# fmidev/RoadSurf

Measured on AMD Instinct MI355X. Metric: point_timesteps_per_s, higher is better.
Workload: dtype f64

## Files before the change

roadsurf_amd/csrc/rs_api.hip:

```cpp
#include <hip/hip_runtime.h>
#include <atomic>
#include <cmath>
#include <cstdarg>
#include <cstdio>
#include <cstdlib>
#include <cstring>
#include <mutex>
#include <utility>
#include <vector>

#include "../../include/roadsurf.h"
#include "rs_kernels.h"
#include "rs_ens_table.hpp"
#include "rs_period_rule.hpp"
#include "rs_devutil.hpp"
#include <cstdint>
#include <algorithm>
#include "rs_consts_dev.h"
#include "rs_state.h"

static thread_local char g_err[512] = "";

static int set_err(const char *fmt, ...) {
  va_list ap;
// ... 1282 lines not shown
  dst->wave_tab_valid = false;
  return 0;
}

int rs_hip_clock_probe(int32_t device, void *out, uint32_t spin_us, void *stream) {
  if (!out) return set_err("rs_hip_clock_probe: null output");
  HIP_OK(hipSetDevice(device));
  HIP_OK(rs_launch_clock_probe(static_cast<uint64_t *>(out), spin_us, (hipStream_t)stream));
  return 0;
}

int64_t rs_hip_failed_count(RsPlan *pl) {
  if (!pl) return -1;
  if (hipSetDevice(pl->device) != hipSuccess) return -1;
  unsigned long long h = 0;
  if (pl->f32) {
    std::vector<float> row((size_t)pl->np_pad);
    if (hipMemcpyAsync(row.data(), (const char *)pl->state + (size_t)RS_ST_FAILED * pl->np_pad * sizeof(float),
                       row.size() * sizeof(float), hipMemcpyDeviceToHost, pl->stream) != hipSuccess)
      return -1;
    if (hipStreamSynchronize(pl->stream) != hipSuccess) return -1;
    for (int64_t q = 0; q < pl->npoints; ++q) h += row[(size_t)q] != 0.f ? 1 : 0;
    return (int64_t)h;
  }
  if (hipMemsetAsync(pl->counter, 0, sizeof(h), pl->stream) != hipSuccess) return -1;
  if (rs_launch_count_failed(pl->state, pl->np_pad, pl->npoints, pl->counter, pl->stream) !=
      hipSuccess)
    return -1;
  if (hipMemcpyAsync(&h, pl->counter, sizeof(h), hipMemcpyDeviceToHost, pl->stream) != hipSuccess)
    return -1;
  if (hipStreamSynchronize(pl->stream) != hipSuccess) return -1;
  return (int64_t)h;
}

int rs_hip_first_failed_index(RsPlan *pl, int32_t *out) {
  if (!pl || !out) return set_err("rs_hip_first_failed_index: bad arguments");
  HIP_OK(hipSetDevice(pl->device));
  const size_t esz = pl->f32 ? sizeof(float) : sizeof(double);
  std::vector<char> row((size_t)pl->np_pad * esz);
  HIP_OK(hipMemcpyAsync(row.data(), (const char *)pl->state + (size_t)RS_ST_FAILED * pl->np_pad * esz,
                        row.size(), hipMemcpyDeviceToHost, pl->stream));
  std::vector<int32_t> order;
  if (pl->order) {
    order.resize((size_t)pl->np_pad);
    HIP_OK(hipMemcpyAsync(order.data(), pl->order, order.size() * sizeof(int32_t), hipMemcpyDeviceToHost,
                          pl->stream));
  }
  HIP_OK(hipStreamSynchronize(pl->stream));
  for (int64_t s = 0; s < pl->npoints; ++s) {
    const double v = pl->f32 ? (double)reinterpret_cast<const float *>(row.data())[s]
                             : reinterpret_cast<const double *>(row.data())[s];
    const int64_t p = pl->order ? order[(size_t)s] : s;
    if (p >= 0 && p < pl->npoints) out[p] = (int32_t)v;
  }
  return 0;
}

int rs_hip_sync(RsPlan *pl) {
  if (!pl) return set_err("rs_hip_sync: null plan");
  HIP_OK(hipSetDevice(pl->device));
  HIP_OK(hipStreamSynchronize(pl->stream));
  return 0;
}

static int64_t div_mismatch(RsPlan *pl, int which) {
  if (!pl) return -1;
  if (hipSetDevice(pl->device) != hipSuccess) return -1;
  unsigned long long n[3] = {0, 0, 0};
  if (rs_read_div_mismatch(n, pl->stream) != hipSuccess) return -1;
  return which == 1 ? (int64_t)(n[1] + n[2]) : (int64_t)n[0];
}
int64_t rs_hip_div_mismatch_count(RsPlan *pl) { return div_mismatch(pl, 0); }
int64_t rs_hip_div_special_count(RsPlan *pl) { return div_mismatch(pl, 1); }
int rs_hip_div_samples(RsPlan *pl, double *out) {
  if (!pl || !out) return set_err("rs_hip_div_samples: bad arguments");
  HIP_OK(hipSetDevice(pl->device));
  HIP_OK(rs_read_div_samples(out, pl->stream));
  return 0;
}

int rs_hip_bl_stats(RsPlan *pl, int64_t *out) {
  if (!pl || !out) return set_err("rs_hip_bl_stats: bad arguments");
  HIP_OK(hipSetDevice(pl->device));
  unsigned long long v[57];
  HIP_OK(rs_read_bl_stats(v, pl->stream));
  for (int k = 0; k < 57; ++k) out[k] = (int64_t)v[k];
  return 0;
}

int rs_hip_division_mode(void) {
#if defined(RS_IEEE_DIV)
  return 0;
#elif defined(RS_DIV_CHECK)
  return 2;
#else
  return 1;
#endif
}

int rs_hip_test_math(RsPlan *pl, int32_t fn, int64_t n, const double *x, double *y) {
  if (!pl || !x || !y || n < 1 || fn < 0 || fn > 3) return set_err("rs_hip_test_math: bad arguments");
  HIP_OK(hipSetDevice(pl->device));
  HIP_OK(rs_launch_math_test(fn, n, x, y, pl->stream));
  return 0;
}

int rs_hip_synth_knots(RsPlan *pl, const RsSynthSpec *spec, double *knots, int32_t k0,
                       int32_t nknots) {
  if (!pl || !spec || !knots || nknots < 1 || k0 < 0)
    return set_err("rs_hip_synth_knots: bad arguments");
  if (nknots > 65535) return set_err("rs_hip_synth_knots: at most 65535 knots per call");
  HIP_OK(hipSetDevice(pl->device));
  rs::KnotArgs a;
  a.spec = *spec;
  a.knots = knots;
  a.npoints = pl->npoints;
  a.np_pad = pl->np_pad;
  a.k0 = k0;
  HIP_OK(rs_launch_knots(a, nknots, pl->stream));
  return 0;
}

static int expand_forcing(RsPlan *pl, const RsSynthSpec *spec, const double *knots, int32_t k0,
                          int32_t nknots, const RsForcing *f, int32_t t0, int32_t nsteps, void *stream,
                          const int32_t *gather) {
  if (!pl || !spec || !knots || !f) return set_err("rs_hip_expand_forcing: bad arguments");
  if (check_forcing(pl, f, "rs_hip_expand_forcing")) return -1;
  if (nsteps < 1 || nsteps > 65535 || t0 < 1)
    return set_err("rs_hip_expand_forcing: 1 <= nsteps <= 65535, t0 >= 1");
  const int32_t spk = spec->steps_per_knot;
  if (spk < 1) return set_err("rs_hip_expand_forcing: steps_per_knot < 1");
  const int32_t kfirst = (t0 - 1) / spk;
  const int32_t tlast = t0 + nsteps - 2;
  const int32_t klast = tlast / spk + ((tlast % spk) ? 1 : 0);
  if (kfirst < k0 || klast >= k0 + nknots)
    return set_err("rs_hip_expand_forcing: need knots %d..%d, buffer has %d..%d", kfirst, klast,
                   k0, k0 + nknots - 1);
  if (f->hour_pstride) return set_err("rs_hip_expand_forcing: hour must be a shared axis");
  HIP_OK(hipSetDevice(pl->device));
  rs::ExpandArgs a;
  a.f = *f;
  a.knots = knots;
  a.npoints = pl->npoints;
  a.np_pad = pl->np_pad;
  a.k0 = k0;
  a.t0 = t0;
  a.spk = spk;
  a.start_hour = spec->start_hour;
  a.kfirst = kfirst;
  a.nsteps = nsteps;
  a.r_spk = 1.0 / (double)spk;
  a.gather = gather;
  if (pl->f32) {
    if (f->depth) return set_err("rs_hip_expand_forcing: fp32 windows carry no depth stream");
    HIP_OK(rs32_launch_expand(a, (t0 + nsteps - 2) / spk - kfirst + 1, (hipStream_t)stream));
  } else {
    HIP_OK(rs_launch_expand(a, (t0 + nsteps - 2) / spk - kfirst + 1, (hipStream_t)stream));
  }
  return 0;
}

int rs_hip_expand_forcing_on(RsPlan *pl, const RsSynthSpec *spec, const double *knots, int32_t k0,
                             int32_t nknots, const RsForcing *f, int32_t t0, int32_t nsteps,
                             void *stream) {
  return expand_forcing(pl, spec, knots, k0, nknots, f, t0, nsteps, stream, nullptr);
}

int rs_hip_expand_forcing(RsPlan *pl, const RsSynthSpec *spec, const double *knots, int32_t k0,
                          int32_t nknots, const RsForcing *f, int32_t t0, int32_t nsteps) {
// ... 14 lines not shown
```

roadsurf_amd/csrc/rs_consts_dev.h:

```cpp
#pragma once
#include <cmath>
#include <cstdlib>
#include "../../include/roadsurf.h"

struct RsConstantsDev : RsConstants {
  double meltDen;
  double r_3600, r_3364, r_1000, r_IceMax, r_twoDT, r_DTSecs, r_meltDen, r_logUstar, r_logCond;
  int32_t bareFastOk;
  int32_t precFastOk;
  double chk[8];
  const double *relax_tab;
  const double *cpl_tab;
  double capDZF[RS_MAX_LAYERS + 2];
  double hs1F;
  double hcw[8];
  struct LayerRow {
    double capDZF, condDZ, DyC, dryCap, WCont, pad[3];
  } lk[RS_MAX_LAYERS + 2];
  double stabSafe;
};

static inline double rs_stab_safe(double logMom, double logHeat) {
  if (!(logMom > 0.0 && logMom < HUGE_VAL && logHeat > 0.0 && logHeat < HUGE_VAL)) return NAN;
  const double psih = std::fmin(logHeat / 2.0, logMom / 1.2);
  const double sq = 2.0 * std::exp(psih / 2.0) - 1.0;
  return (1.0 - sq * sq) / 16.0;
}

static inline void rs_consts_dev_fill(const RsConstants &c, RsConstantsDev &d) {
  static_cast<RsConstants &>(d) = c;
  d.meltDen = c.WatMHeat * c.WatDens;
  d.r_3600 = 1.0 / 3600.0;
  d.r_3364 = 1.0 / 3364.0;
  d.r_1000 = 1.0 / 1000.0;
  d.r_IceMax = 1.0 / 1.5;
  d.r_twoDT = 1.0 / c.twoDT;
  d.r_DTSecs = 1.0 / c.DTSecs;
  d.r_meltDen = 1.0 / d.meltDen;
  d.r_logUstar = 1.0 / c.logUstar;
  d.r_logCond = 1.0 / c.logCond;
  const float chk[8] = {100.0f, -0.1f, -90.0f, 120.0f, -1.0f, 4000.0f, 1000.0f, 500.0f};
  for (int i = 0; i < 8; ++i) d.chk[i] = (double)chk[i];
  d.relax_tab = nullptr;
  d.cpl_tab = nullptr;
  for (int j = 0; j < RS_MAX_LAYERS + 2; ++j) {
    d.lk[j].capDZF = 0.0;
    d.lk[j].condDZ = c.condDZ[j];
    d.lk[j].DyC = c.DyC[j];
    d.lk[j].dryCap = c.dryCap[j];
    d.lk[j].WCont = c.WCont[j];
    d.lk[j].pad[0] = d.lk[j].pad[1] = d.lk[j].pad[2] = 0.0;
  }
  {
    const float h[8] = {-0.0050f, 0.0079f, 1000.0028f, 0.0000102f, 0.0017169f, 0.11516f, 3.4739f, 4217.2f};
    for (int i = 0; i < 8; ++i) d.hcw[i] = (double)h[i];
  }
  for (int j = 0; j < RS_MAX_LAYERS + 2; ++j) d.capDZF[j] = 0.0;
  d.hs1F = 0.0;
  for (int j = 1; j <= c.NLayers && j <= RS_MAX_LAYERS; ++j) {
    const volatile double chwt = 920.0 * 2100.0;
    const volatile double wc = c.WCont[j] * chwt;
    const volatile double vsh = c.dryCap[j] + wc;
    const volatile double den = c.DyC[j] * vsh;
    d.capDZF[j] = -(1.0 / den);
    d.lk[j].capDZF = d.capDZF[j];
    if (j == 1) {
      const volatile double num = vsh * c.HSfac1;
      d.hs1F = num / c.twoDT;
    }
  }
  d.stabSafe = rs_stab_safe(c.logMom, c.logHeat);
  d.bareFastOk = (c.MaxWatmms >= 0.0 && c.MaxSnowmms >= 0.0 && c.MaxIcemms >= 0.0 && c.MaxDepmms >= 0.0) ? 1 : 0;
  d.precFastOk = (c.MinPrecmm >= 0.0) ? 1 : 0;
}

static inline const char *rs_consts_domain_error(const RsConstants &c) {
  const double lo = 1e-30, hi = 1e30;
  auto pos = [&](double x) { return x > lo && x < hi; };
  auto mag = [&](double x) { return (x > lo && x < hi) || (x < -lo && x > -hi); };
  if (!pos(c.DTSecs) || !pos(c.twoDT)) return "DTSecs";
  if (!mag(c.logUstar)) return "logUstar = log(ZRefW/ZMom)";
  if (!mag(c.logCond)) return "logCond = log(ZRefT/ZHeat)";
  if (!(c.logMom > -hi && c.logMom < hi) || !(c.logHeat > -hi && c.logHeat < hi)) return "logMom/logHeat";
  if (!pos(c.VK_Const)) return "VK_Const";
  if (!pos(c.LVap) || !pos(c.LFus)) return "LVap/LFus";
  if (!pos(c.WatMHeat * c.WatDens)) return "WatMHeat*WatDens";
  if (!pos(c.HSfac1)) return "layer grid (ZDpth(2)-ZDpth(1))";
  for (int j = 1; j <= c.NLayers; ++j) {
    if (!pos(c.DyC[j])) return "DyC (layer grid)";
    if (!(c.dryCap[j] >= 0.0) || !(c.WCont[j] >= 0.0) || !pos(c.dryCap[j] + c.WCont[j] * 1.9e6))
      return "layer heat capacity (vsh/Poro/WCont)";
    if (!(c.ZDpth[j + 1] - c.ZDpth[j] > lo)) return "layer grid (ZDpth)";
  }
  return nullptr;
}

#include <cmath>
#include <vector>
static inline std::vector<double> rs_decay_table(const RsConstants &c, bool on, double den) {
  std::vector<double> t;
  const double dt = c.DTSecs;
  if (!on || !(dt == std::floor(dt)) || !(dt * ((double)c.SimLen + 1.0) < 9.0e15)) return t;
  t.resize((size_t)c.SimLen + 1);
  for (int32_t d = 0; d <= c.SimLen; ++d) t[(size_t)d] = std::exp(-((dt * d) - (dt * 0)) / den);
  return t;
}
static inline std::vector<double> rs_relax_table(const RsConstants &c) {
  return rs_decay_table(c, c.use_relaxation != 0, (double)(4.f * 3600.f));
}
static inline std::vector<double> rs_cpl_table(const RsConstants &c) {
  return rs_decay_table(c, c.use_coupling != 0 && c.cplReduction > 1e-30 && c.cplReduction < 1e30,
                        c.cplReduction);
}
```

roadsurf_amd/csrc/rs_kernels.hip:

```cpp
#include <hip/hip_runtime.h>
#include <cstdlib>
#include "rs_physics.hpp"
#include "rs_state.h"
#include "rs_synth.h"
#include "rs_kernels.h"

#ifndef RS_CPL_WAVES
#define RS_CPL_WAVES 2
#endif
#ifndef RS_REGIME_WINDOW
#define RS_REGIME_WINDOW 30
#endif

namespace rs {

constexpr int kBlock = RS_BLOCK;

typedef RsConstantsDev __attribute__((address_space(4))) ConstsAS;
template <class Args>
__device__ __forceinline__ const ConstsAS &consts_of(Args a) {
  return *(const ConstsAS *)a->consts;
}

template <int NL, int NREG>
// ... 729 lines not shown
        } else {
          s.tsurf = (T.get(1) + T.get(2)) / R4(2.0);
        }
      }
      const double tair = q.tair;
      auto qs = q;
      if (SKY) {
        const int64_t row = (int64_t)k * ka->f.t_stride + row0;
        const LaneOff L(lane);
        double sw_dir = L.ld(ka->f.sw_dir + row), lw_net = L.ld(ka->f.lw_net + row);
        if (i < c.SimLen) {
          if (sky_on && sky_limits_bad(sw_dir, lw_net)) fail_at(i);
          sw_dir = sky_clamp_direct(sw_dir, q.sw);
        }
        if (sky_on) {
          int64_t hstride;
          const double *hrow = horizon_row(ka, sky.hcol, hstride);
          if (!sky_view_radiation(ka->f.sun + (int64_t)k * RS_SUN_COLS, sky.sinlat, sky.coslat, sky.lonrad, sky.coslon,
                                  sky.sinlon, sky.skyv, ka->pp.albedo_surroundings, hrow, hstride, qs.sw, sw_dir, qs.lw,
                                  lw_net))
            fail_at(i);
        }
        sky_write_back(ka, k, row0, sky_on, sw_dir, qs.sw, qs.lw, [&](double *base, double v) { L.st(base, v); });
      }
      const Fluxes fx = model_step_fluxes_prepped<SCORE ? 1 : 2>(c, mt, s, qs, cp);
      if (SCORE) {
        score += (fx.trips & 63) - 5;
        if ((fx.trips & 64) && k >= nsteps - RS_REGIME_WINDOW) score |= 1 << 30;
      } else if (k == nsteps - 1) {
        score = fx.trips;
      }
      if (LATE) t3 = mail.v[k & 1][1][ml];
      model_step_ground<RegProfile<2>, RegProfile<2>, false>(c, s, T, t3, tair, fx, R4(-9999.9), cp);
      if (owrite) {
        if (OUTIDX && ka->out_index) store_outputs<true, false>(ka, orow, row0, lane, s, true);
        else store_outputs<false, true>(ka, orow, row0, lane, s, true);
      }
      if (s.failed) blank_rows(REPLAY && cpl_ce + 1 > i + 1 ? cpl_ce + 1 : i + 1);
      if (CPL && cpl_on && i < c.SimLen && i == cpl_ce)
        cpl_window_end(ka->state, ka->np_pad, row0 + lane, cw, s, cpl_swcorr, cpl_lwcorr, cpl_lastobs, parked);
    }
    mail.failed[(k & 1) ^ 1][ml] = (s.failed || (CPL && (parked || (i + 1) != next_i))) ? 1u : 0u;
    mail.v[(k & 1) ^ 1][0][ml] = T.get(2);
    if (!OUTIDX) {
      if (owrite) {
        orow_next += ostride;
        owait = odec - 1;
      } else {
        --owait;
      }
    }
    duo_meet();
  }
  if (CPL && live) a.state[(int64_t)RS_ST_CPL_RESUME * a.np_pad + p] = (double)next_i;
  if (live) {
    double *st = a.state;
    const int64_t np = a.np_pad;
    uint32_t le = ml;
    if (LATE) asm volatile("" : "+v"(le));
    const int64_t p = LATE ? row0 + le : row0 + lane;
    st[(int64_t)(RS_ST_TMP0 + 0) * np + p] = T.get(1);
    st[(int64_t)(RS_ST_TMP0 + 1) * np + p] = T.get(2);
    st[(int64_t)RS_ST_TNW1 * np + p] = s.tnw1;
    st[(int64_t)RS_ST_TNW2 * np + p] = s.tnw2;
    st[(int64_t)RS_ST_TSURF * np + p] = s.tsurf;
    st[(int64_t)RS_ST_WAT * np + p] = s.wat;
    st[(int64_t)RS_ST_SNOW * np + p] = s.snow;
    st[(int64_t)RS_ST_ICE * np + p] = s.ice;
    st[(int64_t)RS_ST_ICE2 * np + p] = s.ice2;
    st[(int64_t)RS_ST_DEP * np + p] = s.dep;
    st[(int64_t)RS_ST_Q2MELT * np + p] = s.q2melt;
    st[(int64_t)RS_ST_T4MELT * np + p] = s.t4melt;
    st[(int64_t)RS_ST_ALBEDO * np + p] = s.albedo;
    st[(int64_t)RS_ST_VERYCOLD * np + p] = s.verycold ? 1.0 : 0.0;
    st[(int64_t)RS_ST_BLSCORE * np + p] = SCORE ? bl_score_key(score, s) : (double)score;
  }
}

template <bool FULL>
struct KnotLerp {
  double v0[FULL ? 7 : 6], dv[FULL ? 7 : 6];
  int32_t ph1;
  int32_t spk, k, r, hour, night;
  double span, r_spk;
};
template <bool FULL>
__device__ __forceinline__ void knot_begin(KernArgs ka, KnotLerp<FULL> &K, int32_t i0) {
  K.spk = ka->spk;
  {
    const uint64_t u = (uint64_t)__double_as_longlong((double)K.spk);
    const uint32_t lo = __builtin_amdgcn_readfirstlane((uint32_t)u), hi = __builtin_amdgcn_readfirstlane((uint32_t)(u >> 32));
    K.span = __longlong_as_double((long long)(((uint64_t)hi << 32) | lo));
  }
  K.r_spk = ka->r_spk;
  const int32_t t = i0 - 1;
  K.k = __builtin_amdgcn_readfirstlane(t / K.spk);
  K.r = t - K.k * K.spk;
  K.hour = 0;
  K.night = 0;
}
template <bool FULL>
__device__ __forceinline__ Forcing knot_forcing(KernArgs ka, int64_t col, bool live, KnotLerp<FULL> &K,
                                                int32_t &kcur, int32_t i) {
  const int32_t k = K.k, r = K.r;
  int32_t ph0 = 0;
  if (k != kcur) {
    kcur = k;
    const ConstsAS &c = consts_of(ka);
    K.hour = (k + ka->start_hour) % 24;
    const bool night = ((double)K.hour >= c.NightOn) || ((double)K.hour <= c.NightOff);
    K.night = __builtin_amdgcn_readfirstlane(night ? 1 : 0);
    const int fld[7] = {0, 2, 3, 4, 5, 6, 1};
    const int64_t np = ka->np_pad;
    const double *ka_ = ka->knots + ((int64_t)(k - ka->knot_k0) * RS_KNOT_FIELDS) * np + col;
    const bool has_b = (k + 1 - ka->knot_k0) < ka->knot_n;
    const double *kb_ = ka_ + (int64_t)RS_KNOT_FIELDS * np;
#pragma unroll
    for (int q = 0; q < (FULL ? 7 : 6); ++q) {
      K.v0[q] = live ? ka_[(int64_t)fld[q] * np] : 0.0;
      const double v1 = (live && has_b) ? kb_[(int64_t)fld[q] * np] : K.v0[q];
      K.dv[q] = v1 - K.v0[q];
    }
    ph0 = live ? (int32_t)ka_[8 * np] : 0;
    K.ph1 = (live && has_b) ? (int32_t)kb_[8 * np] : ph0;
  }
  const int32_t spk = FULL ? ka->spk : K.spk;
  const double secs = (double)r, span = FULL ? (double)spk : K.span, r_spk = FULL ? ka->r_spk : K.r_spk;
  Forcing f;
  f.tair = K.v0[0] + rs_div_u(secs * K.dv[0], span, r_spk);
  f.vz = K.v0[1] + rs_div_u(secs * K.dv[1], span, r_spk);
  f.rhz = K.v0[2] + rs_div_u(secs * K.dv[2], span, r_spk);
  f.prec = K.v0[3] + rs_div_u(secs * K.dv[3], span, r_spk);
  f.sw = K.v0[4] + rs_div_u(secs * K.dv[4], span, r_spk);
  f.lw = K.v0[5] + rs_div_u(secs * K.dv[5], span, r_spk);
  f.phase = (r == 0) ? ph0 : K.ph1;
  f.hour = K.hour;
  f.tdew = 0.0;
  f.tsurfobs = R4(-9999.9);
  if (FULL) {
    f.tdew = K.v0[6] + rs_div_u(secs * K.dv[6], span, r_spk);
    if (i == 1 && live) f.tsurfobs = (ka->knots + ((int64_t)(k - ka->knot_k0) * RS_KNOT_FIELDS + 7) * ka->np_pad)[col];
  }
  f.depth = R4(-9999.9);
  K.r = r + 1;
  if (K.r == spk) {
    K.r = 0;
    K.k = k + 1;
  }
  return f;
}

enum { FSET_ALL = 0, FSET_GROUND = 1, FSET_SKY = 2 };
__device__ __forceinline__ constexpr int raw_nfields(int fset) { return fset == FSET_ALL ? 8 : fset == FSET_GROUND ? 6 : 4; }
__device__ __forceinline__ constexpr int raw_field_of(int fset, int q) {
  return fset == FSET_SKY ? (q == 0 ? RAW_SW : q == 1 ? RAW_LW : q == 2 ? RAW_SWDIR : RAW_LWNET)
                          : (q == 0 ? RAW_TAIR : q == 1 ? RAW_VZ : q == 2 ? RAW_RHZ : q == 3 ? RAW_PREC
                             : q == 4 ? RAW_TDEW : q == 5 ? RAW_OBS : q == 6 ? RAW_SW : RAW_LW);
}
constexpr int kRawObs = 5;
template <int NF>
struct RawLerp {
  double v0[NF], dv[NF];
  uint64_t mode;
  int32_t single;
  int32_t seg, seg_end;
  uint32_t mixed, imask;
  uint32_t wsel;
};

__device__ __forceinline__ double raw_slow_value(KernArgs ka, int fld, int64_t col, int32_t i) {
  const double thr = raw_threshold(fld);
  double v = raw_miss();
  const int nsrc = ka->raw.nsrc;
  const int64_t np = ka->raw.np_pad;
  for (int s = 0; s < nsrc; ++s) {
    const double *x = ka->raw.src[s].fld[fld];
    if (!x) continue;
    const RawPlanStep st = raw_plan_at(ka->raw.src[s].plan, i);
    if (st.kind == RAW_NONE) continue;
    const double a = x[(int64_t)st.rp * np + col], b = x[(int64_t)(st.rp + 1) * np + col];
    double vs;
    if (raw_source_value(st, a, b, thr, vs)) v = vs;
  }
  return v;
}

template <int FSET>
__device__ __forceinline__ void raw_resolve(KernArgs ka, int64_t col, bool live, RawLerp<raw_nfields(FSET)> &R) {
  constexpr int NF = raw_nfields(FSET);
  const RawSeg __attribute__((address_space(4))) *sg =
      (const RawSeg __attribute__((address_space(4))) *)ka->raw.segs + R.seg;
  R.seg_end = sg->i1;
  const int32_t i0 = sg->i0;
  const int nsrc = ka->raw.nsrc;
  const int64_t np = ka->raw.np_pad;
  uint64_t mode = 0;
  uint32_t mixed = 0u, imask = 0u, wsel = 0u;
  for (int s = 0; s < nsrc; ++s)
    if (sg->kind[s] == RAW_INTERP) imask |= 1u << s;
#pragma unroll
  for (int q = 0; q < NF; ++q) {
    const int fld = raw_field_of(FSET, q);
    const double thr = raw_threshold(fld);
    int32_t wl = 4;
    bool okl = true;
    double a_w = raw_miss(), d_w = 0.0;
    for (int s = 0; s < nsrc; ++s) {
      const double *x = ka->raw.src[s].fld[fld];
      const int32_t kind = sg->kind[s], rp = sg->rp[s];
      if (!x || kind == RAW_NONE) continue;
      const double *xa = x + (int64_t)rp * np + col;
      const double a = *xa;
      if (kind == RAW_COPY) {
        if (a > thr) {
          wl = 4;
          a_w = a;
// ... 109 lines not shown
    for (int q = 0; q < NF; ++q)
      if (slow & (1u << q)) val[q] = raw_slow_value(ka, raw_field_of(FSET, q), col, t);
  }
}

template <int FSET>
__device__ __forceinline__ Forcing raw_forcing(KernArgs ka, int64_t col, bool live, bool rejected,
                                               RawLerp<raw_nfields(FSET)> &R, int32_t i, bool need_obs) {
  double val[raw_nfields(FSET)];
  raw_values<FSET>(ka, col, live, R, i, need_obs, val);
  Forcing f;
  f.tair = rejected ? raw_miss() : val[0];
  f.vz = val[1];
  f.rhz = val[2];
  f.prec = val[3];
  f.tdew = val[4];
  f.tsurfobs = need_obs ? val[kRawObs] : raw_miss();
  f.sw = FSET == FSET_ALL ? val[FSET == FSET_ALL ? 6 : 0] : 0.0;
  f.lw = FSET == FSET_ALL ? val[FSET == FSET_ALL ? 7 : 0] : 0.0;
  f.phase = -9999;
  f.hour = ((const int32_t __attribute__((address_space(4))) *)ka->raw.hour)[i - 1];
  f.depth = raw_miss();
  return f;
}

enum { SRC_WINDOW = 0, SRC_KNOTS = 1, SRC_RAW = 2 };
template <int NL, int SRC = SRC_WINDOW, bool FULL = false, bool SKYG = false, bool CPL = false, bool REPLAY = false>
__device__ __forceinline__ void duo_ground(const MathTab &mt, DuoMailT<FULL ? PR_FULL : PR_LEAN> &mail, const StepArgs &a) {
  constexpr bool KNOTS = SRC == SRC_KNOTS, RAW = SRC == SRC_RAW;
  static_assert(FULL || !CPL, "coupling belongs to the FULL feature set");
  static_assert(!RAW || FULL, "the driver's series carry the FULL feature set");
  static_assert(!SKYG || RAW, "a sky wave exists only where the forcing is made from the raw series");
  static_assert(!REPLAY || (CPL && RAW && !SKYG), "replay rounds in this flavour: raw series, no sky view");
  static_assert(!KNOTS || (!CPL && !REPLAY), "the knot-reading source steps every index of the launch in order");
  KernArgs ka = kernargs();
  const uint32_t ml = threadIdx.x & 63u;
  const int64_t listed = REPLAY ? (int64_t)blockIdx.x * 64 + ml : 0;
  const int64_t row0 = REPLAY ? 0 : a.wave_start ? (int64_t)a.wave_start[blockIdx.x] : (int64_t)blockIdx.x * 64;
  const uint32_t lane = REPLAY ? (listed < a.cpl_nlist ? (uint32_t)a.cpl_list[listed] : 0u) : ml;
  const int64_t p = row0 + lane;
  const bool live = REPLAY ? listed < a.cpl_nlist
                           : a.wave_start ? (int32_t)lane < a.wave_cnt[blockIdx.x] : p < a.npoints;
  double Tg[NL - 2];
#pragma unroll
  for (int j = 3; j <= NL; ++j) Tg[j - 3] = live ? a.state[(int64_t)(RS_ST_TMP0 + j - 1) * a.np_pad + p] : 0.0;
  constexpr bool LATE = !FULL;
  const double tbot = (live && !LATE) ? ka->pp.tbottom[p] : 0.0;
  mail.v[0][1][ml] = Tg[0];
  const int32_t nsteps = ka->nsteps, t0 = ka->t0;
  int32_t initlen = 0;
  bool relax = false;
  double relax_dt = 0, relax_dv = 0, relax_dr = 0;
  auto relax_targets = [&](double &tairR, double &vzR, double &rhR) {
    tairR = (double)(float)ka->pp.tair_relax[p];
    vzR = (double)(float)ka->pp.vz_relax[p];
    rhR = (double)(float)ka->pp.rh_relax[p];
  };
  if (FULL && live) {
    initlen = ka->pp.initlen ? ka->pp.initlen[p] : 0;
    if (consts_of(ka).use_relaxation && ka->pp.tair_relax) {
      double tairR, vzR, rhR;
      relax_targets(tairR, vzR, rhR);
      relax = !(tairR < R4(-100.0) || tairR > R4(100.0) || vzR < R4(0.0) || vzR > R4(100.0) ||
                rhR < R4(0.0) || rhR > 110);
      relax_dt = tairR - a.state[(int64_t)RS_ST_TAIR_END * a.np_pad + p];
      relax_dv = vzR - a.state[(int64_t)RS_ST_VZ_END * a.np_pad + p];
      relax_dr = rhR - a.state[(int64_t)RS_ST_RH_END * a.np_pad + p];
    }
  }
  int32_t cpl_cs = 0x7fffffff, cpl_ce = 0x7ffffff0;
  if (CPL && live) {
    const int32_t cidx = ka->pp.coupling_index ? ka->pp.coupling_index[p] : 0;
    if (consts_of(ka).use_coupling && ka->pp.coupling_index && !(ka->pp.coupling_tsurf[p] < -100 || cidx < 1)) {
      cpl_cs = ((double)cidx <= consts_of(ka).cplLenR) ? 1 : cidx - consts_of(ka).cplLenI;
      cpl_ce = cidx;
    }
  }
  const int64_t rcol_ = (RAW && live) ? (ka->raw.col ? (int64_t)ka->raw.col[p] : p) : 0;
  bool anchor_due = false;
  double anchor_t = 0, anchor_v = 0, anchor_r = 0;
  double obs_cur = R4(-9999.9);
  KnotLerp<FULL> klerp;
  klerp.night = 0;
  auto prep = [&](const ConstsAS &c, const Forcing &f, int32_t in, double &obs) -> ForcingPrep {
    if (!FULL) return forcing_prep<KNOTS>(c, mt, f, in, in < c.SimLen, klerp.night != 0);
    bool bad;
    const bool has_tdew = RAW ? true : KNOTS ? (ka->knots_tdew & 2) != 0 : ka->f.tdew != nullptr;
    double vz = forcing_prep_head(c, f, in, in < c.SimLen, has_tdew, bad);
    double tair = f.tair, rhz = f.rhz;
    obs = R4(-9999.9);
    if (in < c.SimLen) {
      if ((in <= initlen || c.force_tsurf) && f.tsurfobs > R4(-100.0) && (!CPL || in < cpl_cs)) obs = f.tsurfobs;
      if (relax) {
        if (in == initlen) {
          double tairR, vzR, rhR;
          relax_targets(tairR, vzR, rhR);
          relax_dt = tairR - tair;
          relax_dv = vzR - vz;
          relax_dr = rhR - rhz;
          anchor_due = true;
          anchor_t = tair;
          anchor_v = vz;
          anchor_r = rhz;
        }
        if (in > initlen) {
          double e;
          const uint32_t d = (uint32_t)(in - initlen);
          if (c.relax_tab && d <= (uint32_t)c.SimLen) {
            e = ((const double *)c.relax_tab)[d];
          } else {
            const double den = (double)(4.f * 3600.f);
            e = rs_exp(mt, rs_div(-((c.DTSecs * in) - (c.DTSecs * initlen)), den));
          }
          tair = tair - relax_dt * e;
          vz = vz - relax_dv * e;
          rhz = rhz - relax_dr * e;
          if (rhz > R4(100.)) rhz = R4(100.0);
        }
      }
    }
    ForcingPrep q = forcing_prep_tail<KNOTS>(c, mt, f, tair, vz, rhz, bad, klerp.night != 0);
    q.tsurfobs = obs;
    if (REPLAY && live && in == cpl_cs && in < c.SimLen) {
      Forcing g = Forcing();
      const int32_t tb = cpl_ce;
      g.tair = ka->raw.status && ka->raw.status[rcol_] != 0 ? raw_miss() : raw_slow_value(ka, RAW_TAIR, rcol_, tb);
      g.vz = raw_slow_value(ka, RAW_VZ, rcol_, tb);
      g.rhz = raw_slow_value(ka, RAW_RHZ, rcol_, tb);
      g.prec = raw_slow_value(ka, RAW_PREC, rcol_, tb);
      g.sw = raw_slow_value(ka, RAW_SW, rcol_, tb);
      g.lw = raw_slow_value(ka, RAW_LW, rcol_, tb);
      g.tdew = raw_slow_value(ka, RAW_TDEW, rcol_, tb);
      q.bad_rw = check_values_forcing(c, g) | (g.tdew < -90) | (g.tdew > R4(100.0));
    }
    return q;
  };
  Forcing nxt = Forcing();
  int32_t kcur = -1;
  const int32_t kcol32 = (KNOTS && LATE && live) ? (ka->knot_gather ? ka->knot_gather[p] : (int32_t)lane) : 0;
  const int64_t kcol0 = (KNOTS && LATE && !ka->knot_gather) ? row0 : 0;
  const int64_t kcol = LATE ? 0 : (KNOTS && live) ? (ka->knot_gather ? (int64_t)ka->knot_gather[p] : p) : 0;
  constexpr int FSET = SKYG ? FSET_GROUND : FSET_ALL;
  RawLerp<raw_nfields(FSET)> rlerp;
  const int64_t rcol = rcol_;
  const bool rejected = RAW && live && ka->raw.status && ka->raw.status[rcol] != 0;
  auto obs_wanted = [&](const ConstsAS &c, int32_t in) -> bool {
    return c.force_tsurf || __builtin_amdgcn_ballot_w64(live && in <= initlen) != 0ull;
  };
  if (RAW) {
    rlerp.seg = ka->raw.seg0;
    raw_resolve<FSET>(ka, rcol, live, rlerp);
  }
  {
    const ConstsAS &c0 = consts_of(ka);
    if (KNOTS) {
      knot_begin<FULL>(ka, klerp, t0);
      nxt = knot_forcing<FULL>(ka, LATE ? kcol0 + kcol32 : kcol, live, klerp, kcur, t0);
    } else if (RAW) nxt = raw_forcing<FSET>(ka, rcol, live, rejected, rlerp, t0, obs_wanted(c0, t0));
    else if (live) nxt = load_forcing<FULL, true>(ka, row0, lane, 0);
    duo_put_prep<FULL, SKYG>(mail, 0, ml, prep(c0, nxt, t0, obs_cur));
  }
  duo_meet();
  for (int32_t kv = 0; kv < nsteps; ++kv) {
    asm volatile("" : "+s"(ka));
    const ConstsAS &c = consts_of(ka);
    const int32_t k = __builtin_amdgcn_readfirstlane(kv);
    if (!KNOTS && !RAW && k + 1 < nsteps && live) nxt = load_forcing<FULL, true>(ka, row0, lane, k + 1);
    double t2 = mail.v[k & 1][0][ml];
    const double tbot_k = !LATE ? tbot : live ? LaneOff(lane).ld(ka->pp.tbottom + row0) : 0.0;
    if (REPLAY && !mail.failed[k & 1][ml] && t0 + k == cpl_cs && t0 + k < c.SimLen && live) {
      const double *sv = ka->state + (int64_t)RS_ST_CPL_SAVE_TMP0 * ka->np_pad + p;
      const int64_t np = ka->np_pad;
      double cur = sv[(int64_t)2 * np];
      double Gprev = c.lk[2].condDZ * (cur - sv[np]);
#pragma unroll
      for (int j = 3; j <= NL; ++j) {
        const double tnext = (j == NL) ? tbot : sv[(int64_t)j * np];
        const double stale = Tg[j - 3];
        Tg[j - 3] = layer_step(c, j, cur, stale, tnext, Gprev, nullptr);
        cur = tnext;
      }
    } else
    if (!mail.failed[k & 1][ml]) {
      if (CPL && !REPLAY && t0 + k == cpl_cs && t0 + k < c.SimLen && live) {
#pragma unroll
        for (int j = 3; j <= NL; ++j) ka->state[(int64_t)(RS_ST_CPL_SAVE_TMP0 + j - 1) * ka->np_pad + p] = Tg[j - 3];
      }
      if (FULL) {
        if (obs_cur > R4(-100.0)) t2 = obs_cur;
        if (anchor_due && live) {
          double *st = ka->state;
          st[(int64_t)RS_ST_TAIR_END * ka->np_pad + p] = anchor_t;
          st[(int64_t)RS_ST_VZ_END * ka->np_pad + p] = anchor_v;
          st[(int64_t)RS_ST_RH_END * ka->np_pad + p] = anchor_r;
        }
      }
      double Gprev = c.lk[2].condDZ * (Tg[0] - t2);
#pragma unroll
      for (int j = 3; j <= NL; ++j) {
        const double tj = Tg[j - 3];
        const double tnext = (j == NL) ? tbot_k : Tg[j - 2];
        Tg[j - 3] = layer_step(c, j, tj, tj, tnext, Gprev, nullptr);
      }
    }
// ... 610 lines not shown
```

roadsurf_amd/csrc/rs_math.hpp:

```cpp
#pragma once
#include <hip/hip_runtime.h>
#include "rs_glibc_tables.h"

namespace rs {

static __constant__ uint64_t c_gl_exp_tab[256] = {0};
static __constant__ uint64_t c_gl_log_tab[256] = {0};

enum { RS_K_EXP_SHIFT, RS_K_EXP_C2, RS_K_EXP_C4, RS_K_LOG_A1, RS_K_LOG_A3, RS_K_LOG_B1,
       RS_K_LOG_B4, RS_K_LOG_B7, RS_K_COUNT };
static __constant__ uint64_t c_gl_coef[RS_K_COUNT] = {
    RS_GL_EXP_SHIFT, RS_GL_EXP_C2, RS_GL_EXP_C4, RS_GL_LOG_A1,
    RS_GL_LOG_A3,    RS_GL_LOG_B1, RS_GL_LOG_B4, RS_GL_LOG_B7};

enum { RS_S_EXP_INVLN2N, RS_S_EXP_NEGLN2HIN, RS_S_EXP_NEGLN2LON, RS_S_EXP_C3, RS_S_EXP_C5, RS_S_PAD0, RS_S_PAD1, RS_S_PAD2,
       RS_S_LOG_LN2HI, RS_S_LOG_A2, RS_S_LOG_LN2LO, RS_S_LOG_A4, RS_S_LOG_A0, RS_S_PAD3, RS_S_PAD4, RS_S_PAD5,
       RS_S_LOG_B2, RS_S_LOG_B5, RS_S_LOG_B8, RS_S_LOG_B3, RS_S_LOG_B6, RS_S_LOG_B9, RS_S_LOG_B10, RS_S_LOG_B0,
       RS_S_COUNT };
static __constant__ uint64_t c_gl_scoef[RS_S_COUNT] = {
    RS_GL_EXP_INVLN2N, RS_GL_EXP_NEGLN2HIN, RS_GL_EXP_NEGLN2LON, RS_GL_EXP_C3, RS_GL_EXP_C5, 0, 0, 0,
    RS_GL_LOG_LN2HI, RS_GL_LOG_A2, RS_GL_LOG_LN2LO, RS_GL_LOG_A4, RS_GL_LOG_A0, 0, 0, 0,
    RS_GL_LOG_B2, RS_GL_LOG_B5, RS_GL_LOG_B8, RS_GL_LOG_B3, RS_GL_LOG_B6, RS_GL_LOG_B9, RS_GL_LOG_B10, RS_GL_LOG_B0};
typedef const double __attribute__((address_space(4))) *MathCoef;

struct MathTab {
  const uint64_t *expT;
  const double *logT;
  const double *K;
  MathCoef S;
};

#define RS_MATH_LDS_DOUBLES (512 + RS_K_COUNT)

__device__ __forceinline__ MathTab fill_math_tables(double *lds) {
  uint64_t *w = reinterpret_cast<uint64_t *>(lds);
  for (int i = threadIdx.x; i < RS_MATH_LDS_DOUBLES; i += blockDim.x)
    w[i] = (i < 256) ? c_gl_exp_tab[i] : (i < 512) ? c_gl_log_tab[i - 256] : c_gl_coef[i - 512];
  MathTab t;
  t.expT = w;
  t.logT = lds + 256;
  t.K = lds + 512;
  t.S = (MathCoef)c_gl_scoef;
  asm volatile("" : "+s"(t.S));
  return t;
}

static __device__ unsigned long long g_div_mismatch[3] = {0ull, 0ull, 0ull};
#define RS_BL_NSTATS 57
static __device__ unsigned long long g_bl_stats[RS_BL_NSTATS];
#define RS_DIV_SAMPLES 64
static __device__ double g_div_samples[RS_DIV_SAMPLES][4];
__device__ __forceinline__ void div_check_note(double q, double f, double a = 0.0, double b = 0.0) {
  if (__double_as_longlong(q) == __double_as_longlong(f) || (q != q && f != f)) return;
  const bool special = !(__builtin_fabs(q) < __builtin_inf()) || !(__builtin_fabs(f) < __builtin_inf());
  const int kind = special ? 1 : (q == f ? 2 : 0);
  const unsigned long long k = atomicAdd(&g_div_mismatch[kind], 1ull);
  if (kind == 0 && k < RS_DIV_SAMPLES) {
    g_div_samples[k][0] = a;
    g_div_samples[k][1] = b;
    g_div_samples[k][2] = q;
    g_div_samples[k][3] = f;
  }
}

__device__ __forceinline__ double div_bare(double a, double b) {
  double r = __builtin_amdgcn_rcp(b);
  double e = __builtin_fma(-b, r, 1.0);
#ifdef RS_DIV_TWO_NEWTON
  r = __builtin_fma(r, e, r);
  e = __builtin_fma(-b, r, 1.0);
  r = __builtin_fma(r, e, r);
#else
  e = __builtin_fma(e, e, e);
  r = __builtin_fma(r, e, r);
#endif
  const double q = a * r;
  const double rem = __builtin_fma(-b, q, a);
  return __builtin_fma(rem, r, q);
}

__device__ __forceinline__ double sqrt_bare(double x) {
  const double y = __builtin_amdgcn_rsq(x);
  double g = x * y;
  double h = 0.5 * y;
  const double r = __builtin_fma(-h, g, 0.5);
  g = __builtin_fma(g, r, g);
  h = __builtin_fma(h, r, h);
  double d = __builtin_fma(-g, g, x);
  g = __builtin_fma(d, h, g);
  d = __builtin_fma(-g, g, x);
  return __builtin_fma(d, h, g);
}

__device__ __forceinline__ double rs_div(double a, double b) {
#if defined(RS_IEEE_DIV)
  return a / b;
#elif defined(RS_DIV_CHECK)
  const double q = a / b, f = div_bare(a, b);
  div_check_note(q, f, a, b);
  return q;
#else
  return div_bare(a, b);
#endif
}

__device__ __forceinline__ double rs_sqrt(double x) {
#if defined(RS_IEEE_DIV)
  return ::sqrt(x);
#elif defined(RS_DIV_CHECK)
  const double q = ::sqrt(x), f = sqrt_bare(x);
  div_check_note(q, f, x, 0.0);
  return q;
#else
  return sqrt_bare(x);
#endif
}

__device__ __forceinline__ double rs_div_u(double a, double b, double rb) {
#if defined(RS_IEEE_DIV)
  return a / b;
#else
  const double q0 = a * rb;
  const double rem = __builtin_fma(-b, q0, a);
  const double f = __builtin_fma(rem, rb, q0);
#if defined(RS_DIV_CHECK)
  const double q = a / b;
  div_check_note(q, f, a, b);
  return q;
#else
  return f;
#endif
// ... 165 lines not shown
```

roadsurf_amd/csrc/rs_physics_body.inc:

```
namespace RS_NS {

struct Scalars {
  RS_REAL tnw1, tnw2;
  RS_REAL tsurf;
  RS_REAL wat, snow, ice, ice2, dep;
  RS_REAL q2melt, t4melt, albedo;
  RS_REAL tair_end, vz_end, rh_end;
  bool verycold, failed;
};

struct Forcing {
  RS_REAL tair, tdew, vz, rhz, prec, sw, lw, tsurfobs, depth;
  int32_t phase, hour;
};

template <class Prof>
__device__ __forceinline__ RS_REAL temp_at_depth(const RS_CONSTS &c, const Prof &T, RS_REAL tbot,
                                                RS_REAL depth) {
  const int N = T.nlayers();
  if (rs_fabs(depth - R4(0.0)) < R4(0.00001)) return T.get(1);
  if (depth > c.ZDpth[N + 1]) return tbot;
  RS_REAL r = 0.0;
  bool found = false;
#pragma unroll
// ... 645 lines not shown
__device__ __forceinline__ bool check_values_tsurf(const RS_CONSTS &c, RS_REAL tsurf) {
  return rs_fabs(tsurf) > RS_CHK(c, 0, R4(100.0));
}

__device__ __forceinline__ RS_REAL forcing_prep_head(const RS_CONSTS &c, const Forcing &f, int32_t i,
                                                     bool checked, bool has_tdew, bool &bad) {
  RS_REAL vz = f.vz;
  if (i == 1 && vz < R4(0.4)) vz = R4(0.4);
  bad = false;
  if (checked) {
    Forcing chk = f;
    chk.vz = vz;
    bad = check_values_forcing(c, chk);
    if (has_tdew) bad = bad | (f.tdew < -90) | (f.tdew > R4(100.0));
  }
  return vz;
}

__device__ __forceinline__ RS_REAL air_vapour_pressure(const MathTab &mt, RS_REAL tair, RS_REAL rhz) {
  const RS_REAL aa = (tair < 0) ? R4(21.875) : R4(17.269);
  const RS_REAL ba = (tair < 0) ? R4(265.5) : R4(237.3);
  const RS_REAL ESat = R4(0.61078) * rs_exp(mt, rs_dv<false>(aa * tair, tair + ba));
  return rs_min_num_one(R4(0.01) * rhz) * ESat;
}

template <bool NIGHT_U = false>
__device__ __forceinline__ ForcingPrep forcing_prep_tail(const RS_CONSTS &c, const MathTab &mt, const Forcing &f,
                                                         RS_REAL tair, RS_REAL vz, RS_REAL rhz, bool bad,
                                                         bool night_u = false) {
  ForcingPrep q;
  RS_REAL prec_ts = RS_DIVC(f.prec, (RS_REAL)3600.0, r_3600) * c.DTSecs;
  q.bad = bad;
  {
    Scalars z;
    z.wat = R4(0.0);
    z.snow = R4(0.0);
#ifdef RS_BL_STATS
    {
      const unsigned long long act = __builtin_amdgcn_ballot_w64(true);
      const bool dry = __builtin_amdgcn_ballot_w64(prec_ts == R4(0.0)) == act;
      if ((unsigned long long)__builtin_ctzll(act) == (unsigned long long)(threadIdx.x & 63u)) {
        atomicAdd(&rs::g_bl_stats[17], 1ull);
        if (!dry) atomicAdd(&rs::g_bl_stats[18], 1ull);
      }
    }
#endif
    if (!(RS_PREC_FAST(c) && rs_wave_all(prec_ts == R4(0.0))))
      precipitation_to_storage(c, mt, z, f.phase, prec_ts, tair, rhz);
    q.rain = z.wat;
    q.snow = z.snow;
  }
  const RS_REAL calmN = c.CalmLimNgt, calmD = c.CalmLimDay, fricN = c.TrfFricNgt, fricD = c.TrFfricDay;
  const bool night = NIGHT_U ? night_u : ((RS_REAL)f.hour >= c.NightOn) || ((RS_REAL)f.hour <= c.NightOff);
  const RS_REAL calm = night ? calmN : calmD;
  q.trffric = night ? fricN : fricD;
  q.night = night;
  if (vz < calm) vz = calm;
  q.tair = tair;
  q.vz = vz;
  q.rhz = rhz;
  const RS_REAL TaK = tair + R4(273.15);
  q.AirDens = rs_dv<false>(R4(100000.0), R4(287.05) * TaK);
  const RS_REAL dK = (TaK - R4(250.0)) * (TaK - R4(250.0));
  q.AirHCap = R4(1005.0) + RS_DIVC(dK, R4(3364.), r_3364);
  const RS_REAL AirVCap = q.AirHCap * q.AirDens;
  q.PsychC = R4(0.1) * (R4(0.00063) * TaK + R4(0.47496));
  q.den0 = AirVCap * (tair + R4(273.15));
  q.vkvz = c.VK_Const * vz;
  q.avk = AirVCap * c.VK_Const;
#ifndef RS_EAIR_SURFACE
  q.EAir = air_vapour_pressure(mt, tair, rhz);
#endif
  q.sw = f.sw;
  q.lw = f.lw;
  return q;
}

template <bool NIGHT_U = false>
__device__ __forceinline__ ForcingPrep forcing_prep(const RS_CONSTS &c, const MathTab &mt, const Forcing &f,
                                                    int32_t i, bool checked, bool night_u = false) {
  bool bad;
  const RS_REAL vz = forcing_prep_head(c, f, i, checked, false, bad);
  return forcing_prep_tail<NIGHT_U>(c, mt, f, f.tair, vz, f.rhz, bad, night_u);
}

#ifdef RS_BL_STATS
struct BlStatsStep {
  unsigned long long act;
  bool first;
};
__device__ __forceinline__ BlStatsStep bl_stats_step() {
  const unsigned long long act = __builtin_amdgcn_ballot_w64(true);
  const bool first = (unsigned long long)__builtin_ctzll(act) == (unsigned long long)(threadIdx.x & 63u);
  if (first) {
    atomicAdd(&rs::g_bl_stats[0], 1ull);
    atomicAdd(&rs::g_bl_stats[1], (unsigned long long)__builtin_popcountll(act));
  }
  return BlStatsStep{act, first};
}
__device__ __forceinline__ void bl_stats_pass(const BlStatsStep &st, int j, RS_REAL h0, const BlVar &x) {
  const unsigned long long act = st.act;
  const bool first = st.first;
  {
    const bool uns = !(x.PSIH > R4(0.0)), far = x.PSIH < R4(-0.1254);
    const unsigned long long mu = __builtin_amdgcn_ballot_w64(uns), mf = __builtin_amdgcn_ballot_w64(far),
                             ma = __builtin_amdgcn_ballot_w64(true);
    if ((unsigned long long)__builtin_ctzll(ma) == (unsigned long long)(threadIdx.x & 63u)) {
      atomicAdd(&rs::g_bl_stats[19], 1ull);
      atomicAdd(&rs::g_bl_stats[48], (unsigned long long)__builtin_popcountll(ma));
      atomicAdd(&rs::g_bl_stats[46], (unsigned long long)__builtin_popcountll(mu));
      atomicAdd(&rs::g_bl_stats[47], (unsigned long long)__builtin_popcountll(mf));
      if (mu) atomicAdd(&rs::g_bl_stats[20], 1ull);
      if (mf && (mu & ~mf)) atomicAdd(&rs::g_bl_stats[21], 1ull);
      if (mu && (ma & ~mu)) atomicAdd(&rs::g_bl_stats[22], 1ull);
      if (mf) atomicAdd(&rs::g_bl_stats[23], 1ull);
    }
  }
  if (j >= 2 && j <= 4) {
    const bool same = __double_as_longlong((double)h0) == __double_as_longlong((double)x.PSIH);
    const unsigned long long ms = __builtin_amdgcn_ballot_w64(same);
    if (first) {
      if (ms == act) atomicAdd(&rs::g_bl_stats[j], 1ull);
      atomicAdd(&rs::g_bl_stats[3 + j], (unsigned long long)__builtin_popcountll(ms));
    }
  }
}
__device__ __forceinline__ void bl_stats_trips(const BlStatsStep &st, int j) {
  const bool first = st.first;
  {
    const int trips = j > RS_BL_MAXIT ? RS_BL_MAXIT : j;
    int wmax = trips, wsum = trips;
    for (int o = 32; o > 0; o >>= 1) {
      const int other = __shfl_xor(wmax, o, 64);
      wmax = other > wmax ? other : wmax;
      wsum += __shfl_xor(wsum, o, 64);
    }
    auto bin = [](int t) { return t <= 8 ? t - 5 : t <= 12 ? 4 : t <= 20 ? 5 : t < 40 ? 6 : 7; };
    for (int b = 0; b < 8; ++b) {
      const unsigned long long mb = __builtin_amdgcn_ballot_w64(bin(trips) == b);
      if (first && mb) atomicAdd(&rs::g_bl_stats[32 + b], (unsigned long long)__builtin_popcountll(mb));
    }
    {
      const int nh = __builtin_popcountll(__builtin_amdgcn_ballot_w64(trips > 20));
      if (first && nh > 0) atomicAdd(&rs::g_bl_stats[40 + (nh == 1 ? 0 : nh <= 3 ? 1 : nh <= 7 ? 2 : nh <= 15 ? 3 : nh <= 31 ? 4 : 5)], 1ull);
    }
    if (first) {
      atomicAdd(&rs::g_bl_stats[9], (unsigned long long)wsum);
      atomicAdd(&rs::g_bl_stats[8], (unsigned long long)wmax);
      atomicAdd(&rs::g_bl_stats[24 + bin(wmax)], 1ull);
    }
  }
}
#endif

#ifdef RS_BL_LAST
template <class Q>
__device__ __forceinline__ RS_REAL le_numerator(const MathTab &mt, RS_REAL tsurf, const Q &q) {
  const RS_REAL as = (tsurf < 0) ? R4(21.875) : R4(17.269);
  const RS_REAL bs = (tsurf < 0) ? R4(265.5) : R4(237.3);
  const RS_REAL ESurf = R4(0.61078) * rs_exp(mt, rs_dv<false>(as * tsurf, tsurf + bs));
#ifdef RS_EAIR_SURFACE
  const RS_REAL EAir = air_vapour_pressure(mt, q.tair, q.rhz_late());
#else
  const RS_REAL EAir = q.EAir;
#endif
  return q.AirVCap * (ESurf - EAir);
// ... 328 lines not shown
```

Baseline: 27.93 billion.

## Precompute per-knot-interval facts to skip forcing checks, precip, and interpolation

When a new forcing knot interval is loaded, the kernel checks both endpoint values against the validity thresholds (shrunk slightly by a margin), the calm-wind limit, and exact-zero precip and shortwave, then reduces each result to a wave-wide flag. The per-timestep forcing prep reads these flags to skip range checks, precipitation-to-storage, the calm-wind clamp, and the prec/sw interpolation. This removes per-step branching and arithmetic from the hot path, at the cost of more work at knot boundaries and reliance on linear interpolation keeping values between the endpoints.

```diff
diff --git a/roadsurf_amd/csrc/rs_api.hip b/roadsurf_amd/csrc/rs_api.hip
--- a/roadsurf_amd/csrc/rs_api.hip
+++ b/roadsurf_amd/csrc/rs_api.hip
@@ -1388,9 +1388,9 @@
 int rs_hip_bl_stats(RsPlan *pl, int64_t *out) {
   if (!pl || !out) return set_err("rs_hip_bl_stats: bad arguments");
   HIP_OK(hipSetDevice(pl->device));
-  unsigned long long v[57];
+  unsigned long long v[62];
   HIP_OK(rs_read_bl_stats(v, pl->stream));
-  for (int k = 0; k < 57; ++k) out[k] = (int64_t)v[k];
+  for (int k = 0; k < 62; ++k) out[k] = (int64_t)v[k];
   return 0;
 }
 
diff --git a/roadsurf_amd/csrc/rs_consts_dev.h b/roadsurf_amd/csrc/rs_consts_dev.h
--- a/roadsurf_amd/csrc/rs_consts_dev.h
+++ b/roadsurf_amd/csrc/rs_consts_dev.h
@@ -18,7 +18,14 @@
     double capDZF, condDZ, DyC, dryCap, WCont, pad[3];
   } lk[RS_MAX_LAYERS + 2];
   double stabSafe;
+  double chkIn[8];
+  double calmInNgt, calmInDay;
 };
+
+#define RS_KNOT_MARGIN 0x1p-20
+static inline double rs_calm_in(double calm) {
+  return (calm >= -4000.0 && calm <= 4000.0) ? calm + RS_KNOT_MARGIN : HUGE_VAL;
+}
 
 static inline double rs_stab_safe(double logMom, double logHeat) {
   if (!(logMom > 0.0 && logMom < HUGE_VAL && logHeat > 0.0 && logHeat < HUGE_VAL)) return NAN;
@@ -41,6 +48,10 @@
   d.r_logCond = 1.0 / c.logCond;
   const float chk[8] = {100.0f, -0.1f, -90.0f, 120.0f, -1.0f, 4000.0f, 1000.0f, 500.0f};
   for (int i = 0; i < 8; ++i) d.chk[i] = (double)chk[i];
+  for (int i = 0; i < 8; ++i)
+    d.chkIn[i] = (i == 1 || i == 2 || i == 4) ? d.chk[i] + RS_KNOT_MARGIN : d.chk[i] - RS_KNOT_MARGIN;
+  d.calmInNgt = rs_calm_in(c.CalmLimNgt);
+  d.calmInDay = rs_calm_in(c.CalmLimDay);
   d.relax_tab = nullptr;
   d.cpl_tab = nullptr;
   for (int j = 0; j < RS_MAX_LAYERS + 2; ++j) {
diff --git a/roadsurf_amd/csrc/rs_kernels.hip b/roadsurf_amd/csrc/rs_kernels.hip
--- a/roadsurf_amd/csrc/rs_kernels.hip
+++ b/roadsurf_amd/csrc/rs_kernels.hip
@@ -835,6 +835,7 @@
   double v0[FULL ? 7 : 6], dv[FULL ? 7 : 6];
   int32_t ph1;
   int32_t spk, k, r, hour, night;
+  int32_t facts;
   double span, r_spk;
 };
 template <bool FULL>
@@ -851,6 +852,7 @@
   K.r = t - K.k * K.spk;
   K.hour = 0;
   K.night = 0;
+  K.facts = 0;
 }
 template <bool FULL>
 __device__ __forceinline__ Forcing knot_forcing(KernArgs ka, int64_t col, bool live, KnotLerp<FULL> &K,
@@ -868,12 +870,28 @@
     const double *ka_ = ka->knots + ((int64_t)(k - ka->knot_k0) * RS_KNOT_FIELDS) * np + col;
     const bool has_b = (k + 1 - ka->knot_k0) < ka->knot_n;
     const double *kb_ = ka_ + (int64_t)RS_KNOT_FIELDS * np;
+#ifndef RS_NO_KNOT_INTERVAL_FACTS
+    const int lo[7] = {2, 4, 1, 1, 1, 1, 2}, hi[7] = {0, 0, 3, 7, 5, 6, 0};
+    const double calm_in = night ? c.calmInNgt : c.calmInDay;
+    bool tame = true, dry = false, dark = false, windy = false;
+#endif
 #pragma unroll
     for (int q = 0; q < (FULL ? 7 : 6); ++q) {
       K.v0[q] = live ? ka_[(int64_t)fld[q] * np] : 0.0;
       const double v1 = (live && has_b) ? kb_[(int64_t)fld[q] * np] : K.v0[q];
       K.dv[q] = v1 - K.v0[q];
-    }
+#ifndef RS_NO_KNOT_INTERVAL_FACTS
+      const double v0 = K.v0[q];
+      tame = tame && v0 > c.chkIn[lo[q]] && v0 < c.chkIn[hi[q]] && v1 > c.chkIn[lo[q]] && v1 < c.chkIn[hi[q]];
+      if (q == 1) windy = v0 >= calm_in && v1 >= calm_in && v0 < c.chkIn[0] && v1 < c.chkIn[0];
+      if (q == 3) dry = rs_is_pos_zero(v0) && rs_is_pos_zero(v1);
+      if (q == 4) dark = rs_is_pos_zero(v0) && rs_is_pos_zero(v1);
+#endif
+    }
+#ifndef RS_NO_KNOT_INTERVAL_FACTS
+    K.facts = (rs_wave_all(tame || !live) ? RS_KF_TAME : 0) | (c.precFastOk != 0 && rs_wave_all(dry || !live) ? RS_KF_DRY : 0) |
+              (rs_wave_all(dark || !live) ? RS_KF_DARK : 0) | (rs_wave_all(windy) ? RS_KF_WINDY : 0);
+#endif
     ph0 = live ? (int32_t)ka_[8 * np] : 0;
     K.ph1 = (live && has_b) ? (int32_t)kb_[8 * np] : ph0;
   }
@@ -883,8 +901,29 @@
   f.tair = K.v0[0] + rs_div_u(secs * K.dv[0], span, r_spk);
   f.vz = K.v0[1] + rs_div_u(secs * K.dv[1], span, r_spk);
   f.rhz = K.v0[2] + rs_div_u(secs * K.dv[2], span, r_spk);
+#ifdef RS_NO_KNOT_INTERVAL_FACTS
   f.prec = K.v0[3] + rs_div_u(secs * K.dv[3], span, r_spk);
   f.sw = K.v0[4] + rs_div_u(secs * K.dv[4], span, r_spk);
+#else
+  const int32_t facts = K.facts;
+#ifdef RS_BL_STATS
+  if ((unsigned long long)__builtin_ctzll(__builtin_amdgcn_ballot_w64(true)) == (unsigned long long)(threadIdx.x & 63u)) {
+    atomicAdd(&rs::g_bl_stats[57], 1ull);
+    for (int b = 0; b < 4; ++b)
+      if (facts & (1 << b)) atomicAdd(&rs::g_bl_stats[58 + b], 1ull);
+  }
+#endif
+  f.prec = 0.0;
+  if (!(facts & RS_KF_DRY)) {
+    f.prec = K.v0[3] + rs_div_u(secs * K.dv[3], span, r_spk);
+    asm volatile("" : "+v"(f.prec));
+  }
+  f.sw = 0.0;
+  if (!(facts & RS_KF_DARK)) {
+    f.sw = K.v0[4] + rs_div_u(secs * K.dv[4], span, r_spk);
+    asm volatile("" : "+v"(f.sw));
+  }
+#endif
   f.lw = K.v0[5] + rs_div_u(secs * K.dv[5], span, r_spk);
   f.phase = (r == 0) ? ph0 : K.ph1;
   f.hour = K.hour;
@@ -1160,11 +1199,19 @@
   double obs_cur = R4(-9999.9);
   KnotLerp<FULL> klerp;
   klerp.night = 0;
+  klerp.facts = 0;
   auto prep = [&](const ConstsAS &c, const Forcing &f, int32_t in, double &obs) -> ForcingPrep {
+#ifndef RS_NO_KNOT_INTERVAL_FACTS
+    constexpr bool KFACTS = KNOTS;
+#else
+    constexpr bool KFACTS = false;
+#endif
+    if (!FULL && KFACTS) return forcing_prep_facts<true>(c, mt, f, in, in < c.SimLen, klerp.night != 0, klerp.facts);
     if (!FULL) return forcing_prep<KNOTS>(c, mt, f, in, in < c.SimLen, klerp.night != 0);
     bool bad;
     const bool has_tdew = RAW ? true : KNOTS ? (ka->knots_tdew & 2) != 0 : ka->f.tdew != nullptr;
-    double vz = forcing_prep_head(c, f, in, in < c.SimLen, has_tdew, bad);
+    double vz = KFACTS ? forcing_prep_head_facts(c, f, in, in < c.SimLen, has_tdew, klerp.facts, bad)
+                       : forcing_prep_head(c, f, in, in < c.SimLen, has_tdew, bad);
     double tair = f.tair, rhz = f.rhz;
     obs = R4(-9999.9);
     if (in < c.SimLen) {
@@ -1197,7 +1244,8 @@
         }
       }
     }
-    ForcingPrep q = forcing_prep_tail<KNOTS>(c, mt, f, tair, vz, rhz, bad, klerp.night != 0);
+    ForcingPrep q = KFACTS ? forcing_prep_tail_facts<true>(c, mt, f, tair, vz, rhz, bad, klerp.night != 0, klerp.facts & ~RS_KF_WINDY)
+                           : forcing_prep_tail<KNOTS>(c, mt, f, tair, vz, rhz, bad, klerp.night != 0);
     q.tsurfobs = obs;
     if (REPLAY && live && in == cpl_cs && in < c.SimLen) {
       Forcing g = Forcing();
diff --git a/roadsurf_amd/csrc/rs_math.hpp b/roadsurf_amd/csrc/rs_math.hpp
--- a/roadsurf_amd/csrc/rs_math.hpp
+++ b/roadsurf_amd/csrc/rs_math.hpp
@@ -46,7 +46,7 @@
 }
 
 static __device__ unsigned long long g_div_mismatch[3] = {0ull, 0ull, 0ull};
-#define RS_BL_NSTATS 57
+#define RS_BL_NSTATS 62
 static __device__ unsigned long long g_bl_stats[RS_BL_NSTATS];
 #define RS_DIV_SAMPLES 64
 static __device__ double g_div_samples[RS_DIV_SAMPLES][4];
diff --git a/roadsurf_amd/csrc/rs_physics_body.inc b/roadsurf_amd/csrc/rs_physics_body.inc
--- a/roadsurf_amd/csrc/rs_physics_body.inc
+++ b/roadsurf_amd/csrc/rs_physics_body.inc
@@ -751,6 +751,93 @@
   bool bad;
   const RS_REAL vz = forcing_prep_head(c, f, i, checked, false, bad);
   return forcing_prep_tail<NIGHT_U>(c, mt, f, f.tair, vz, f.rhz, bad, night_u);
+}
+
+enum { RS_KF_TAME = 1, RS_KF_DRY = 2, RS_KF_DARK = 4, RS_KF_WINDY = 8 };
+
+__device__ __forceinline__ RS_REAL forcing_prep_head_facts(const RS_CONSTS &c, const Forcing &f, int32_t i, bool checked,
+                                                           bool has_tdew, int32_t facts, bool &bad) {
+  RS_REAL vz = f.vz;
+  if (i == 1 && vz < R4(0.4)) vz = R4(0.4);
+  bad = false;
+  if (checked && !((facts & RS_KF_TAME) && i > 1)) {
+    Forcing chk = f;
+    chk.vz = vz;
+    bad = check_values_forcing(c, chk);
+    if (has_tdew) bad = bad | (f.tdew < -90) | (f.tdew > R4(100.0));
+  }
+  return vz;
+}
+
+template <bool NIGHT_U = false>
+__device__ __forceinline__ ForcingPrep forcing_prep_tail_facts(const RS_CONSTS &c, const MathTab &mt, const Forcing &f,
+                                                               RS_REAL tair, RS_REAL vz, RS_REAL rhz, bool bad,
+                                                               bool night_u, int32_t facts) {
+  ForcingPrep q;
+  q.bad = bad;
+  q.rain = R4(0.0);
+  q.snow = R4(0.0);
+#ifdef RS_BL_STATS
+  if ((facts & RS_KF_DRY) &&
+      (unsigned long long)__builtin_ctzll(__builtin_amdgcn_ballot_w64(true)) == (unsigned long long)(threadIdx.x & 63u))
+    atomicAdd(&rs::g_bl_stats[17], 1ull);
+#endif
+  if (!(facts & RS_KF_DRY)) {
+    RS_REAL prec_ts = RS_DIVC(f.prec, (RS_REAL)3600.0, r_3600) * c.DTSecs;
+    Scalars z;
+    z.wat = R4(0.0);
+    z.snow = R4(0.0);
+#ifdef RS_BL_STATS
+    {
+      const unsigned long long act = __builtin_amdgcn_ballot_w64(true);
+      const bool dry = __builtin_amdgcn_ballot_w64(prec_ts == R4(0.0)) == act;
+      if ((unsigned long long)__builtin_ctzll(act) == (unsigned long long)(threadIdx.x & 63u)) {
+        atomicAdd(&rs::g_bl_stats[17], 1ull);
+        if (!dry) atomicAdd(&rs::g_bl_stats[18], 1ull);
+      }
+    }
+#endif
+    if (!(RS_PREC_FAST(c) && rs_wave_all(prec_ts == R4(0.0))))
+      precipitation_to_storage(c, mt, z, f.phase, prec_ts, tair, rhz);
+    q.rain = z.wat;
+    q.snow = z.snow;
+  }
+  const RS_REAL calmN = c.CalmLimNgt, calmD = c.CalmLimDay;
+  const RS_REAL fricN = c.TrfFricNgt, fricD = c.TrFfricDay;
+  const bool night = NIGHT_U ? night_u : ((RS_REAL)f.hour >= c.NightOn) || ((RS_REAL)f.hour <= c.NightOff);
+  q.trffric = night ? fricN : fricD;
+  q.night = night;
+  if (!(facts & RS_KF_WINDY)) {
+    const RS_REAL calm = night ? calmN : calmD;
+    if (vz < calm) vz = calm;
+    asm volatile("" : "+v"(vz));
+  }
+  q.tair = tair;
+  q.vz = vz;
+  q.rhz = rhz;
+  const RS_REAL TaK = tair + R4(273.15);
+  q.AirDens = rs_dv<false>(R4(100000.0), R4(287.05) * TaK);
+  const RS_REAL dK = (TaK - R4(250.0)) * (TaK - R4(250.0));
+  q.AirHCap = R4(1005.0) + RS_DIVC(dK, R4(3364.), r_3364);
+  const RS_REAL AirVCap = q.AirHCap * q.AirDens;
+  q.PsychC = R4(0.1) * (R4(0.00063) * TaK + R4(0.47496));
+  q.den0 = AirVCap * (tair + R4(273.15));
+  q.vkvz = c.VK_Const * vz;
+  q.avk = AirVCap * c.VK_Const;
+#ifndef RS_EAIR_SURFACE
+  q.EAir = air_vapour_pressure(mt, tair, rhz);
+#endif
+  q.sw = f.sw;
+  q.lw = f.lw;
+  return q;
+}
+
+template <bool NIGHT_U = false>
+__device__ __forceinline__ ForcingPrep forcing_prep_facts(const RS_CONSTS &c, const MathTab &mt, const Forcing &f,
+                                                          int32_t i, bool checked, bool night_u, int32_t facts) {
+  bool bad;
+  const RS_REAL vz = forcing_prep_head_facts(c, f, i, checked, false, facts, bad);
+  return forcing_prep_tail_facts<NIGHT_U>(c, mt, f, f.tair, vz, f.rhz, bad, night_u, facts);
 }
 
 #ifdef RS_BL_STATS
```

After: 28.20 billion, median of 6. No clear change (+1.0%).
